# endernewton/tf-faster-rcnn

Measured on NVIDIA H100. Metric: images/sec, higher is better.
Workload: dtype f16x3 (fp32-grade: fp16 hi/lo split of both operands, 3 wgmma f16 MMAs per product, fp32 accumulate)

## Files before the change

include/frcnn_b200.h:

```cpp
#ifndef FRCNN_B200_H_
#define FRCNN_B200_H_

#include <stddef.h>
#include <stdint.h>

#ifdef __cplusplus
extern "C" {
#endif

typedef enum {
  FRCNN_OK = 0,
  FRCNN_ERR_CUDA = -1,
  FRCNN_ERR_ARG = -2,
  FRCNN_ERR_NO_DEVICE = -3,
  FRCNN_ERR_DRIVER_ENTRY = -4,
  FRCNN_ERR_CAPACITY = -5
} frcnn_status;

#define FRCNN_NMS_PLUS_ONE 1u
#define FRCNN_NMS_INCLUSIVE 2u
#define FRCNN_NMS_SKIP_DEGENERATE 4u
#define FRCNN_NMS_MODE_CPU_NMS (FRCNN_NMS_PLUS_ONE | FRCNN_NMS_INCLUSIVE)
#define FRCNN_NMS_MODE_GPU_NMS (FRCNN_NMS_PLUS_ONE)
#define FRCNN_NMS_MODE_TF (FRCNN_NMS_SKIP_DEGENERATE)
// ... 21 lines not shown

typedef struct frcnn_conv_plan frcnn_conv_plan;
#define FRCNN_CONV_F16X3 0
#define FRCNN_CONV_TF32X3 1
#define FRCNN_CONV_F16X1 2

typedef struct {
  const float* in_dev;
  const void* w_hi_dev;
  const void* w_lo_dev;
  const float* scale_dev;
  const float* shift_dev;
  const float* residual_dev;
  float* out_dev;
  int n, h, w, cin;
  int cout, kh, kw, stride;
  int pad_t, pad_l;
  int ho, wo;
  int act;
  int block_n;
  int kb_per_chunk;
  int split_k;
  int impl;
  float out_mult;
  const float* in2_dev;
  int cin2;
  float* mean_dev;
  int mean_hw;
} frcnn_conv_desc;

int frcnn_conv_plan_create(frcnn_conv_plan** out, const frcnn_conv_desc* d);
int frcnn_conv_plan_run(const frcnn_conv_plan* p, void* stream);
int frcnn_conv_plan_geometry(const frcnn_conv_desc* d, int sm_count, int* out16);
int frcnn_conv_plan_info(const frcnn_conv_plan* p, int* block_n, int* tile_n, int* tile_h, int* tile_w,
                         int* grid_m, int* grid_n, int* splits, int* smem_bytes);
int frcnn_conv_plan_set_trace(frcnn_conv_plan* p, long long* trace_dev);
void frcnn_conv_plan_destroy(frcnn_conv_plan* p);
int frcnn_debug_watchdog(unsigned int* out16, int reset);

int frcnn_pack_conv_weights(const float* w_hwio_dev, void* w_hi_dev, void* w_lo_dev, int kh, int kw,
                            int cin, int cout, int wexp, void* stream);
int frcnn_pack_conv_weights_tf32(const float* w_hwio_dev, float* w_hi_dev, float* w_lo_dev, int kh, int kw,
                                 int cin, int cout, void* stream);

int frcnn_conv_first(const float* in_dev, const float* w_hwio_dev, const float* scale_dev,
                     const float* shift_dev, float* out_dev, int n, int h, int w, int cout, int k,
                     int stride, int pad_t, int pad_l, int ho, int wo, int act, void* stream);
int frcnn_depthwise3x3(const float* in_dev, const float* w_dev, const float* scale_dev,
                       const float* shift_dev, float* out_dev, int n, int h, int w, int c, int stride,
                       int pad_t, int pad_l, int ho, int wo, int act, void* stream);
int frcnn_max_pool(const float* in_dev, float* out_dev, int n, int h, int w, int c, int k, int stride,
                   int pad_t, int pad_l, int ho, int wo, int pad_is_neg_inf, void* stream);
int frcnn_spatial_mean(const float* in_dev, float* out_dev, int r, int hw, int c, void* stream);

int frcnn_preprocess(const unsigned char* img_dev, int h0, int w0, const double* means3, double fx, double fy,
                     float* blob_dev, int H, int W, void* stream);
int frcnn_preprocess_hflip(const unsigned char* img_dev, int h0, int w0, const double* means3, double fx, double fy,
                           float* blob_dev, int H, int W, void* stream);


int frcnn_rpn_decode(const float* rpn_out_dev, int ld, int delta_col, const float* base_anchors_dev, int num_anchors,
                     int batch, int fh, int fw, int feat_stride, float im_h, float im_w, float* scores_dev,
                     float* props_dev, void* stream);
size_t frcnn_sort_workspace_bytes(int n);
int frcnn_sort_desc(const float* keys_dev, int n, int batch, int* order_dev, float* sorted_keys_dev, void* workspace_dev,
                    size_t workspace_bytes, void* stream);
// ... 73 lines not shown
```

tf_faster_rcnn_b200/_native.py:

```python
import ctypes as C
import os

_HERE = os.path.dirname(os.path.abspath(__file__))
LIB_PATH = os.path.join(_HERE, "libfrcnn_b200_wd.so" if os.environ.get("FRCNN_LIB_VARIANT") == "wd" else "libfrcnn_b200.so")

NMS_PLUS_ONE, NMS_INCLUSIVE, NMS_SKIP_DEGENERATE = 1, 2, 4
NMS_MODE_CPU_NMS = NMS_PLUS_ONE | NMS_INCLUSIVE
NMS_MODE_GPU_NMS = NMS_PLUS_ONE
NMS_MODE_TF = NMS_SKIP_DEGENERATE
ACT_NONE, ACT_RELU, ACT_RELU6 = 0, 1, 2
CONV_F16X3, CONV_TF32X3, CONV_F16X1 = 0, 1, 2
SOFT_NMS_METHODS = {"linear": 0, "gaussian": 1, "hard": 2}
AUG_MAX_VIEWS = 16
BOX_VOTE_METHODS = {"ID": 0, "AVG": 1, "IOU_AVG": 2, "GENERALIZED_AVG": 3, "QUASI_SUM": 4, "TEMP_AVG": 5}
ROI_ALIGN_MAX_SAMPLING = 16
ROI_MAX_POOLED = 16

vp, ci, cf, cu, sz = C.c_void_p, C.c_int, C.c_float, C.c_uint, C.c_size_t
ip, fp = C.POINTER(C.c_int), C.POINTER(C.c_float)


class ConvDesc(C.Structure):
    _fields_ = [("in_dev", vp), ("w_hi_dev", vp), ("w_lo_dev", vp), ("scale_dev", vp), ("shift_dev", vp),
                ("residual_dev", vp), ("out_dev", vp),
                ("n", ci), ("h", ci), ("w", ci), ("cin", ci), ("cout", ci), ("kh", ci), ("kw", ci), ("stride", ci),
                ("pad_t", ci), ("pad_l", ci), ("ho", ci), ("wo", ci), ("act", ci), ("block_n", ci), ("kb_per_chunk", ci), ("split_k", ci),
                ("impl", ci), ("out_mult", cf), ("in2_dev", vp), ("cin2", ci), ("mean_dev", vp), ("mean_hw", ci)]


SIGNATURES = {
    "frcnn_version": (ci, []),
    "frcnn_last_error": (ci, [C.c_char_p, sz]),
    "frcnn_check_device": (ci, [ci]),
    "frcnn_zero_async": (ci, [vp, sz, vp]),
    "frcnn_graph_begin": (ci, [vp]),
    "frcnn_graph_end": (ci, [vp, C.POINTER(vp)]),
    "frcnn_graph_launch": (ci, [vp, vp]),
    "frcnn_graph_destroy": (None, [vp]),
    "frcnn_nms_host": (ci, [ip, ip, fp, ci, ci, cf, ci, cu]),
    "frcnn_nms_sorted_dev": (ci, [vp, ci, cf, cu, ci, vp, vp, vp]),
    "frcnn_conv_plan_create": (ci, [C.POINTER(vp), C.POINTER(ConvDesc)]),
    "frcnn_conv_plan_run": (ci, [vp, vp]),
    "frcnn_conv_plan_geometry": (ci, [C.POINTER(ConvDesc), ci, ip]),
    "frcnn_conv_plan_info": (ci, [vp, ip, ip, ip, ip, ip, ip, ip, ip]),
    "frcnn_conv_plan_set_trace": (ci, [vp, vp]),
    "frcnn_conv_plan_destroy": (None, [vp]),
    "frcnn_debug_watchdog": (ci, [C.POINTER(C.c_uint), ci]),
    "frcnn_pack_conv_weights": (ci, [vp, vp, vp, ci, ci, ci, ci, ci, vp]),
    "frcnn_pack_conv_weights_tf32": (ci, [vp, vp, vp, ci, ci, ci, ci, vp]),
    "frcnn_conv_first": (ci, [vp, vp, vp, vp, vp, ci, ci, ci, ci, ci, ci, ci, ci, ci, ci, ci, vp]),
    "frcnn_depthwise3x3": (ci, [vp, vp, vp, vp, vp, ci, ci, ci, ci, ci, ci, ci, ci, ci, ci, vp]),
    "frcnn_max_pool": (ci, [vp, vp, ci, ci, ci, ci, ci, ci, ci, ci, ci, ci, ci, vp]),
    "frcnn_spatial_mean": (ci, [vp, vp, ci, ci, ci, vp]),
    "frcnn_preprocess": (ci, [vp, ci, ci, C.POINTER(C.c_double), C.c_double, C.c_double, vp, ci, ci, vp]),
    "frcnn_rpn_decode": (ci, [vp, ci, ci, vp, ci, ci, ci, ci, ci, cf, cf, vp, vp, vp]),
    "frcnn_sort_workspace_bytes": (sz, [ci]),
    "frcnn_sort_desc": (ci, [vp, ci, ci, vp, vp, vp, sz, vp]),
    "frcnn_proposals": (ci, [vp, vp, vp, ci, ci, ci, ci, cf, cu, vp, vp, vp, vp, vp]),
    "frcnn_crop_pool": (ci, [vp, ci, ci, ci, ci, vp, ci, ci, ci, vp, vp]),
    "frcnn_roi_align": (ci, [vp, ci, ci, ci, ci, vp, ci, ci, cf, ci, ci, vp, vp]),
    "frcnn_roi_pool": (ci, [vp, ci, ci, ci, ci, vp, ci, ci, cf, vp, vp]),
    "frcnn_cls_finish": (ci, [vp, ci, ci, ci, fp, fp, vp, vp, vp, vp]),
    "frcnn_bbox_decode": (ci, [vp, vp, ci, ci, ci, vp, vp, vp]),
    "frcnn_detect_post_workspace_bytes": (sz, [ci, ci, ci]),
    "frcnn_detect_regions_workspace_bytes": (ci, [ci, ci, ci, C.POINTER(sz)]),
    "frcnn_detect_post": (ci, [vp, vp, vp, ci, ci, ci, cf, cf, cu, ci, ci, vp, vp, ci, vp, vp, vp, vp, sz, vp]),
    "frcnn_soft_nms_host": (ci, [fp, ip, ip, fp, ci, ci, ci, cf, cf, cf, ci]),
    "frcnn_detect_post_soft": (ci, [vp, vp, vp, ci, ci, ci, cf, ci, cf, cf, cf, ci, ci, vp, vp, ci, vp, vp, vp, vp, sz, vp]),
    "frcnn_detect_features": (ci, [vp, vp, vp, ci, ci, ci, ci, ci, vp, vp, vp]),
    "frcnn_detect_regions": (ci, [vp, vp, vp, vp, vp, ci, ci, ci, ci, cf, cu, cf, ci, ci, vp, vp, vp, vp, sz, vp, vp, vp, vp, vp, vp, vp,
                                  vp, vp]),
    "frcnn_regions_attr_embed": (ci, [vp, ci, ci, ci, vp, vp, ci, vp, ci, vp, vp]),
    "frcnn_attr_finish": (ci, [vp, ci, ci, ci, ci, vp, vp, vp, vp, vp]),
    "frcnn_boxes_to_rois": (ci, [vp, vp, vp, ci, ci, vp, vp, vp]),
    "frcnn_preprocess_hflip": (ci, [vp, ci, ci, C.POINTER(C.c_double), C.c_double, C.c_double, vp, ci, ci, vp]),
    "frcnn_aug_union": (ci, [C.POINTER(vp), C.POINTER(vp), C.POINTER(vp), ip, ip, ci, ci, ci, vp, vp, vp, vp, vp]),
# ... 34 lines not shown
```

tf_faster_rcnn_b200/csrc/conv_gemm.cu:

```cuda
#include <cuda_fp16.h>
#include "common.cuh"
#include "../../include/frcnn_b200.h"
#include <stdlib.h>
#include <string.h>

namespace frcnn {

constexpr int BLOCK_M = 128;
constexpr int BLOCK_K = 32;
constexpr int A_TILE_BYTES = BLOCK_M * BLOCK_K * 4;
constexpr int NUM_CONSUMERS = 256;
constexpr int NUM_THREADS = NUM_CONSUMERS + 128;
constexpr int REGS_PRODUCER = 40, REGS_CONSUMER = 232;
constexpr int STAGES = 3;

struct ConvKernelParams {
  float* out;
  const float* residual;
  const float* scale;
  const float* shift;
  int cout, ho, wo, nimg;
  int tn, th, tw;
  int tiles_h, tiles_w;
  int kh, kw, cin, stride, pad_t, pad_l;
  int act;
  int a_box_bytes;
  int kb_per_split;
  int m_tiles, n_tiles, total_units, n_full, splits;
  int raster_n;
  float* ws;
  long long* trace;
  int num_kb_total;
  int cin2;
  float* mean_out;
  float* mean_ws;
  int mean_hw, mean_segs, mean_ld;
};

#ifdef FRCNN_WATCHDOG
#define FRCNN_TRACE(slot, kbv)                                                              \
  do {                                                                                      \
    if (p.trace && blockIdx.x == 0 && (kbv) < 64) p.trace[(kbv) * 8 + (slot)] = clock64(); \
  } while (0)
#else
#define FRCNN_TRACE(slot, kbv) do { } while (0)
#endif

template <int MODE> struct KTraits {
  static constexpr bool TF32 = MODE == FRCNN_CONV_TF32X3;
  static constexpr bool X1 = MODE == FRCNN_CONV_F16X1;
  static constexpr int BOXES = TF32 ? 1 : 2;
  static constexpr int A_BYTES = BOXES * A_TILE_BYTES;
  static constexpr float LO_SCALE = TF32 ? 1.f : 0.00048828125f;
};
template <int BN> constexpr int b_plane_bytes() { return BN * 128; }
template <int BN, int MODE> constexpr int stage_bytes() { return KTraits<MODE>::A_BYTES + 2 * b_plane_bytes<BN>(); }
template <int BN, int MODE> constexpr int smem_bytes() {
  return STAGES * stage_bytes<BN, MODE>() + 1024  + 64 ;
}
constexpr int MEAN_COLS = 64, MEAN_LD = MEAN_COLS + 2;
constexpr int MEAN_SMEM = BLOCK_M * MEAN_LD * 4;
static_assert(smem_bytes<128, FRCNN_CONV_F16X3>() + MEAN_SMEM <= 227 * 1024, "ring exceeds the sm_90 shared-memory limit per block");

struct Unit {
  int w0, h0, n0, nblk, z, kb0, num_kb, slot;
};
__device__ __forceinline__ Unit decode_unit(const ConvKernelParams& p, int u, int num_kb_total) {
  Unit t;
  int tile;
  if (u < p.n_full) { tile = u; t.z = 0; t.slot = -1; }
  else { const int v = u - p.n_full; t.slot = v / p.splits; t.z = v - t.slot * p.splits; tile = p.n_full + t.slot; }
  int mt;
  if (p.raster_n) { t.nblk = tile % p.n_tiles; mt = tile / p.n_tiles; }
  else { mt = tile % p.m_tiles; t.nblk = tile / p.m_tiles; }
  const int tile_w = mt % p.tiles_w;
  const int tile_h = (mt / p.tiles_w) % p.tiles_h;
  const int tile_n = mt / (p.tiles_w * p.tiles_h);
  t.w0 = tile_w * p.tw; t.h0 = tile_h * p.th; t.n0 = tile_n * p.tn;
  if (t.slot < 0) { t.kb0 = 0; t.num_kb = num_kb_total; }
  else { t.kb0 = t.z * p.kb_per_split; t.num_kb = min(p.kb_per_split, num_kb_total - t.kb0); }
  return t;
}

template <int ACT>
__device__ __forceinline__ float apply_act(float a) {
  if (ACT == FRCNN_ACT_RELU) return fmaxf(a, 0.f);
  if (ACT == FRCNN_ACT_RELU6) return fminf(fmaxf(a, 0.f), 6.f);
  return a;
}

template <bool RES, int ACT>
__device__ __forceinline__ float2 finish2(const float2 v, const float2 sc, const float2 sh, const float2 r) {
  float2 y;
  y.x = __fadd_rn(__fmul_rn(v.x, sc.x), sh.x); y.y = __fadd_rn(__fmul_rn(v.y, sc.y), sh.y);
  if (RES) { y.x = __fadd_rn(y.x, r.x); y.y = __fadd_rn(y.y, r.y); }
  y.x = apply_act<ACT>(y.x); y.y = apply_act<ACT>(y.y);
  return y;
}

constexpr int EPI_CHUNK = 8;
template <int BN, bool RES, int ACT>
__device__ __forceinline__ void epilogue_vec(const ConvKernelParams& p, const float (&acc)[BN / 2], const int cbase,
                                             const int pix0, const int pix1) {
  const int cout = p.cout;
  constexpr int NJ = BN / 8;
  constexpr int CH = NJ < EPI_CHUNK ? NJ : EPI_CHUNK;
  static_assert(NJ % CH == 0, "chunking");
  const float* const res0 = RES ? p.residual + (size_t)(pix0 >= 0 ? pix0 : 0) * cout : nullptr;
  const float* const res1 = RES ? p.residual + (size_t)(pix1 >= 0 ? pix1 : 0) * cout : nullptr;
#pragma unroll
  for (int j0 = 0; j0 < NJ; j0 += CH) {
    if (cbase + 8 * j0 >= cout) break;
    float2 sc[CH], sh[CH], r0[CH], r1[CH];
#pragma unroll
// ... 158 lines not shown
  constexpr int kStage = stage_bytes<BN, MODE>();
  constexpr int kPlane = b_plane_bytes<BN>();
  constexpr int NACC = BN / 2;
  static_assert(BN == 64 || BN == 128, "block_n");

  extern __shared__ uint8_t smem_raw[];
  uint8_t* smem = reinterpret_cast<uint8_t*>((reinterpret_cast<uintptr_t>(smem_raw) + 1023) & ~uintptr_t(1023));
  uint64_t* full = reinterpret_cast<uint64_t*>(smem + STAGES * kStage);
  uint64_t* empty = full + STAGES;

  const int warp = threadIdx.x >> 5;
  const int lane = threadIdx.x & 31;
  const int num_kb_total = p.num_kb_total;

  if (threadIdx.x == NUM_CONSUMERS) {
    tma_prefetch_desc(&tmA); tma_prefetch_desc(&tmBhi); tma_prefetch_desc(&tmBlo);
    if (p.cin2) tma_prefetch_desc(&tmA2);
    for (int s = 0; s < STAGES; ++s) { mbar_init(&full[s], 1); mbar_init(&empty[s], NUM_CONSUMERS); }
    mbar_fence_init();
  }
  __syncthreads();
  pdl_launch_dependents();
  pdl_wait();

  if (warp >= NUM_CONSUMERS / 32) {
    reg_dec<REGS_PRODUCER>();
    if (warp == NUM_CONSUMERS / 32 && lane == 0) {
      const int cchunks = p.cin / BLOCK_K;
      const int total1 = p.kh * p.kw * cchunks;
      const int cchunks2 = p.cin2 / BLOCK_K;
      const uint32_t tx = (uint32_t)(T::BOXES * p.a_box_bytes + (T::X1 ? 1 : 2) * kPlane);
      int s = 0; uint32_t ph = 0, kbt = 0;
      for (int u = blockIdx.x; u < p.total_units; u += gridDim.x) {
        const Unit t = decode_unit(p, u, num_kb_total);
#pragma unroll 1
        for (int kb = 0; kb < t.num_kb; ++kb, ++kbt) {
          MBAR_WAIT(&empty[s], ph ^ 1u, 4, kbt);
          uint8_t* st = smem + s * kStage;
          mbar_expect_tx(&full[s], tx);
#pragma unroll
          for (int i = 0; i < T::BOXES; ++i) {
            const int g32 = (t.kb0 + kb) * T::BOXES + i;
            int tap = g32 / cchunks, kc = g32 - tap * cchunks;
            const CUtensorMap* ma = &tmA;
            if (g32 >= total1) {
              tap = 0;
              if (cchunks2) { ma = &tmA2; kc = min(g32 - total1, cchunks2); }
              else kc = cchunks;
            }
            const int r = tap / p.kw, sx = tap - r * p.kw;
            tma_load_4d(st + i * A_TILE_BYTES, ma, &full[s], kc * BLOCK_K, t.w0 * p.stride + sx - p.pad_l,
                        t.h0 * p.stride + r - p.pad_t, t.n0);
          }
          const int kcoord = (t.kb0 + kb) * T::BOXES * BLOCK_K;
          tma_load_2d(st + T::A_BYTES, &tmBhi, &full[s], kcoord, t.nblk * BN);
          if (!T::X1) tma_load_2d(st + T::A_BYTES + kPlane, &tmBlo, &full[s], kcoord, t.nblk * BN);
          FRCNN_TRACE(0, kbt);
          if (++s == STAGES) { s = 0; ph ^= 1u; }
        }
      }
    }
    return;
  }

  reg_inc<REGS_CONSUMER>();
  const int wg = warp >> 2;
  const int q4 = lane & 3;
  const int r0 = wg * 64 + (warp & 3) * 16 + (lane >> 2);
  const uint32_t swz = (uint32_t)(lane >> 2);
  uint32_t aoff[4][2];
#pragma unroll
  for (int j = 0; j < 4; ++j)
#pragma unroll
    for (int h = 0; h < 2; ++h) {
      const int ch = T::TF32 ? j * 8 + h * 4 + q4 : (j & 1) * 16 + h * 8 + 2 * q4;
      const int box = T::TF32 ? 0 : j >> 1;
      aoff[j][h] = (uint32_t)(box * A_TILE_BYTES + r0 * 128) + ((((uint32_t)ch >> 2) ^ swz) << 4) + (((uint32_t)ch & 3u) << 2);
    }
  const uint32_t smem0 = smem_u32(smem);
  int s = 0; uint32_t ph = 0, kbt = 0;
  for (int u = blockIdx.x; u < p.total_units; u += gridDim.x) {
    const Unit t = decode_unit(p, u, num_kb_total);
    float acc[NACC], part[NACC];
#pragma unroll
    for (int i = 0; i < NACC; ++i) { acc[i] = 0.f; part[i] = 0.f; }
#pragma unroll 1
    for (int kb = 0; kb < t.num_kb; ++kb, ++kbt) {
      MBAR_WAIT(&full[s], ph, 1, kbt);
      if (threadIdx.x == 0) FRCNN_TRACE(1, kbt);
      const uint32_t sa = smem0 + (uint32_t)(s * kStage);
      uint32_t ahi[4][4], alo[4][4];
#pragma unroll
      for (int j = 0; j < 4; ++j) {
#pragma unroll
        for (int f = 0; f < 4; ++f) {
          const uint32_t addr = sa + aoff[j][f >> 1] + ((f & 1) ? 1024u : 0u);
          if (T::TF32) {
            float x;
            asm volatile("ld.shared.f32 %0, [%1];" : "=f"(x) : "r"(addr));
            const float hi = to_tf32(x);
            ahi[j][f] = __float_as_uint(hi);
            alo[j][f] = __float_as_uint(to_tf32_fast(__fsub_rn(x, hi)));
          } else {
            float2 x;
            asm volatile("ld.shared.v2.f32 {%0, %1}, [%2];" : "=f"(x.x), "=f"(x.y) : "r"(addr));
            const uint32_t h = pack_f16x2_rn(x.x, x.y);
            const float2 fh = __half22float2(*reinterpret_cast<const __half2*>(&h));
            ahi[j][f] = h;
            alo[j][f] = T::X1 ? 0u : pack_f16x2_rn(__fmul_rn(__fsub_rn(x.x, fh.x), 2048.f), __fmul_rn(__fsub_rn(x.y, fh.y), 2048.f));
          }
        }
      }
      const uint64_t bhi = wgmma_sw128_desc(sa + (uint32_t)T::A_BYTES);
      const uint64_t blo = wgmma_sw128_desc(sa + (uint32_t)(T::A_BYTES + kPlane));
#pragma unroll
      for (int i = 0; i < NACC; ++i) reg_fence(part[i]);
      wgmma_fence();
#pragma unroll
      for (int j = 0; j < 4; ++j) wgmma_rs<BN, MODE>(part, ahi[j], bhi + 2u * j, j > 0 ? 1u : 0u);
      wgmma_commit();
      wgmma_wait_all();
#pragma unroll
      for (int i = 0; i < NACC; ++i) { reg_fence(part[i]); acc[i] = __fadd_rn(acc[i], part[i]); }
      if (!T::X1) {
        wgmma_fence();
#pragma unroll
        for (int j = 0; j < 4; ++j) {
          wgmma_rs<BN, MODE>(part, alo[j], bhi + 2u * j, j > 0 ? 1u : 0u);
          wgmma_rs<BN, MODE>(part, ahi[j], blo + 2u * j, 1u);
        }
        wgmma_commit();
        wgmma_wait_all();
#pragma unroll
        for (int i = 0; i < NACC; ++i) { reg_fence(part[i]); acc[i] = __fmaf_rn(part[i], T::LO_SCALE, acc[i]); }
      }
      mbar_arrive(&empty[s]);
      if (threadIdx.x == 0) FRCNN_TRACE(2, kbt);
      if (++s == STAGES) { s = 0; ph ^= 1u; }
    }
    epilogue_tile<BN>(p, t, acc, r0, q4, reinterpret_cast<float*>(full + 8));
  }
}

template <int BN>
__global__ void __launch_bounds__(256)
tail_reduce_kernel(const ConvKernelParams p) {
  pdl_launch_dependents();
  pdl_wait();
  constexpr int RPB = 256 / (BN / 4);
  constexpr int GROUPS = BLOCK_M / RPB;
  const int slot = blockIdx.x / GROUPS, rgroup = blockIdx.x % GROUPS;
  const int tile = p.n_full + slot;
  const int mt = p.raster_n ? tile / p.n_tiles : tile % p.m_tiles, nblk = p.raster_n ? tile % p.n_tiles : tile / p.m_tiles;
  const int tile_w = mt % p.tiles_w, tile_h = (mt / p.tiles_w) % p.tiles_h, tile_n = mt / (p.tiles_w * p.tiles_h);
  const int rows_img = p.th * p.tw;
  constexpr int C4 = BN / 4;
  static_assert(256 % C4 == 0, "each thread keeps one fixed channel group");
  const float* base = p.ws + (size_t)slot * p.splits * (size_t)(BLOCK_M * BN);
  const bool vec_ok = (p.cout & 3) == 0;
  const int cg = threadIdx.x % C4;
  const int c = nblk * BN + cg * 4;
  if (c >= p.cout) return;
  const float4 sc4 = __ldg(reinterpret_cast<const float4*>(p.scale + c)), sh4 = __ldg(reinterpret_cast<const float4*>(p.shift + c));
  const float sc[4] = {sc4.x, sc4.y, sc4.z, sc4.w}, sh[4] = {sh4.x, sh4.y, sh4.z, sh4.w};
  {
    const int row = rgroup * RPB + threadIdx.x / C4;
    const int dn = row / rows_img, rem = row % rows_img;
    const int n = tile_n * p.tn + dn, h = tile_h * p.th + rem / p.tw, w = tile_w * p.tw + rem % p.tw;
    if (row >= p.tn * rows_img || n >= p.nimg || h >= p.ho || w >= p.wo) return;
    const size_t o = ((((size_t)n * p.ho + h) * p.wo + w)) * p.cout + c;
    float4 rv = make_float4(0.f, 0.f, 0.f, 0.f);
// ... 217 lines not shown
  FRCNN_REQUIRE(bn == 64 || bn == 128, "block_n must be 64 or 128");
  g->bn = bn;
  g->n_tiles = cdiv(d->cout, bn);
  g->tiles = g->m_tiles * g->n_tiles;
  FRCNN_REQUIRE(g->tiles <= 0x3fffffffL, "too many tiles");
  long n_tail = 0; int splits = 1;
  const int num_kb = g->num_kb;
  const int max_split = num_kb * ks / 8 < 8 ? num_kb * ks / 8 : 8;
  if (d->split_k > 1) {
    n_tail = g->tiles; splits = d->split_k;
  } else if (d->split_k == 0 && max_split >= 2) {
    const long rem = g->tiles % sms;
    if (g->tiles <= sms / 2) { if (num_kb * ks >= 16) { n_tail = g->tiles; splits = (int)(sms / g->tiles); } }
    else if (g->tiles > sms && rem > 0 && rem <= sms / 2 && num_kb * ks >= 48) { n_tail = rem; splits = (int)(sms / rem); }
    if (splits > max_split) splits = max_split;
    if (splits < 2) { n_tail = 0; splits = 1; }
  }
  int kbs = cdiv(num_kb, splits);
  splits = cdiv(num_kb, kbs);
  if (splits < 2 || (d->cout & 3) != 0 || mean) { n_tail = 0; splits = 1; kbs = num_kb; }
  FRCNN_REQUIRE(splits <= 64, "bad split_k");
  g->n_tail = n_tail; g->splits = splits; g->kbs = kbs;
  g->total_units = (g->tiles - n_tail) + n_tail * splits;
  FRCNN_REQUIRE(g->total_units <= 0x7fffffffL, "too many work units");
  g->grid = (int)(g->total_units < sms ? g->total_units : sms);
  {
    const char* e = getenv("FRCNN_CONV_RASTER");
    const double a_bytes = (double)d->n * d->h * d->w * (d->cin + d->cin2) * 4.0, b_bytes = (double)d->cout * ktot * 4.0;
    g->raster_n = (e && (e[0] == 'm' || e[0] == 'n')) ? (e[0] == 'n') : (a_bytes > b_bytes && g->n_tiles > 1);
  }
  return OK;
}

extern "C" int frcnn_conv_plan_geometry(const frcnn_conv_desc* d, int sm_count, int* out16) {
  FRCNN_REQUIRE(d && out16, "null argument");
  Geometry g;
  int rc = decide_geometry(d, sm_count, &g);
  if (rc) return rc;
  const int v[16] = {g.bn, g.tn, g.th, g.tw, (int)g.m_tiles, g.n_tiles, (int)g.tiles, (int)g.n_tail, g.splits, g.kbs,
                     (int)g.total_units, g.grid, g.num_kb, g.kpc, g.tiles_h, g.tiles_w};
  for (int i = 0; i < 16; ++i) out16[i] = v[i];
  return OK;
}

extern "C" int frcnn_conv_plan_create(frcnn_conv_plan** out, const frcnn_conv_desc* d) {
  FRCNN_REQUIRE(out && d, "null argument");
  FRCNN_REQUIRE(d->in_dev && d->w_hi_dev && d->w_lo_dev && (d->mean_hw ? d->mean_dev != nullptr : d->out_dev != nullptr),
                "null device pointer");
  FRCNN_REQUIRE(d->cin2 == 0 || d->in2_dev, "cin2=%d without in2_dev", d->cin2);
  int sms = 132;
  { int dev = 0; cudaDeviceProp pr; if (cudaGetDevice(&dev) == cudaSuccess && cudaGetDeviceProperties(&pr, dev) == cudaSuccess && pr.multiProcessorCount > 0) sms = pr.multiProcessorCount; }
  Geometry g;
  int grc = decide_geometry(d, sms, &g);
  if (grc) return grc;
  frcnn_conv_plan* p = (frcnn_conv_plan*)aligned_alloc(64, (sizeof(frcnn_conv_plan) + 63) / 64 * 64);
  if (!p) { set_error("out of host memory"); return ERR_ARG; }
  memset(p, 0, sizeof(*p));
  const int bn = g.bn;
  {
    uint64_t dims[4] = {(uint64_t)d->cin, (uint64_t)g.w, (uint64_t)g.h, (uint64_t)g.n};
    uint64_t strides[3] = {(uint64_t)d->cin * 4, (uint64_t)g.w * d->cin * 4, (uint64_t)g.h * g.w * d->cin * 4};
    uint32_t box[4] = {(uint32_t)BLOCK_K, (uint32_t)(g.tw * d->stride), (uint32_t)(g.th * d->stride), (uint32_t)g.tn};
    uint32_t es[4] = {1, (uint32_t)d->stride, (uint32_t)d->stride, 1};
    int rc = encode_map(&p->tmA, d->in_dev, 4, dims, strides, box, es);
    if (rc) { free(p); return rc; }
    p->tmA2 = p->tmA;
    if (d->cin2 > 0) {
      uint64_t dims2[4] = {(uint64_t)d->cin2, (uint64_t)g.w, (uint64_t)g.h, (uint64_t)g.n};
      uint64_t strides2[3] = {(uint64_t)d->cin2 * 4, (uint64_t)g.w * d->cin2 * 4, (uint64_t)g.h * g.w * d->cin2 * 4};
      rc = encode_map(&p->tmA2, d->in2_dev, 4, dims2, strides2, box, es);
      if (rc) { free(p); return rc; }
    }
  }
  const bool f16 = d->impl != FRCNN_CONV_TF32X3;
  {
    const uint64_t ktot = (uint64_t)d->kh * d->kw * d->cin + d->cin2;
    uint64_t dims[2] = {ktot, (uint64_t)d->cout};
    uint64_t strides[1] = {ktot * (f16 ? 2 : 4)};
    uint32_t box[2] = {(uint32_t)(f16 ? 2 * BLOCK_K : BLOCK_K), (uint32_t)bn};
    uint32_t es[2] = {1, 1};
    const CUtensorMapDataType dt = f16 ? CU_TENSOR_MAP_DATA_TYPE_FLOAT16 : CU_TENSOR_MAP_DATA_TYPE_FLOAT32;
    const CUtensorMapSwizzle sw = CU_TENSOR_MAP_SWIZZLE_128B;
    int rc = encode_map(&p->tmBhi, d->w_hi_dev, 2, dims, strides, box, es, dt, sw);
    if (!rc) rc = encode_map(&p->tmBlo, d->w_lo_dev, 2, dims, strides, box, es, dt, sw);
    if (rc) { free(p); return rc; }
  }
  ConvKernelParams& k = p->kp;
  k.out = d->out_dev; k.residual = d->residual_dev;
  k.cout = d->cout; k.ho = g.ho; k.wo = g.wo; k.nimg = g.n;
  k.tn = g.tn; k.th = g.th; k.tw = g.tw; k.tiles_h = g.tiles_h; k.tiles_w = g.tiles_w;
  k.kh = d->kh; k.kw = d->kw; k.cin = d->cin; k.stride = d->stride; k.pad_t = d->pad_t; k.pad_l = d->pad_l;
  k.act = d->act;
  k.a_box_bytes = g.tn * g.th * g.tw * BLOCK_K * 4;
  k.trace = nullptr;
  k.num_kb_total = g.num_kb;
  k.m_tiles = (int)g.m_tiles; k.n_tiles = g.n_tiles;
  k.kb_per_split = g.kbs; k.splits = g.splits; k.n_full = (int)(g.tiles - g.n_tail);
  k.total_units = (int)g.total_units;
  k.raster_n = g.raster_n;
  k.cin2 = d->cin2;
  k.mean_out = d->mean_hw ? d->mean_dev : nullptr; k.mean_ws = nullptr; k.mean_hw = d->mean_hw; k.mean_ld = g.n_tiles * bn;
  k.mean_segs = d->mean_hw ? (g.tw < cdiv(g.tw - 1, d->mean_hw) + 1 ? g.tw : cdiv(g.tw - 1, d->mean_hw) + 1) : 0;
  k.ws = nullptr; p->ws = nullptr; p->eff = nullptr; p->mean_ws = nullptr; p->n_tail = (int)g.n_tail;
  {
    const int padded = g.n_tiles * bn;
    const float om = f16 ? (d->out_mult != 0.f ? d->out_mult : 1.f) : 1.f;
    cudaError_t e = cudaMalloc(&p->eff, (size_t)2 * padded * sizeof(float));
    if (e != cudaSuccess) { free(p); return cuda_fail(e, "epilogue vectors", __FILE__, __LINE__); }
    prep_epilogue_vectors_kernel<<<cdiv(padded, 256), 256>>>(d->scale_dev, d->shift_dev, om, d->cout, padded, p->eff, p->eff + padded);
    e = cudaGetLastError();
    if (e == cudaSuccess) e = cudaDeviceSynchronize();
    if (e != cudaSuccess) { cudaFree(p->eff); free(p); return cuda_fail(e, "prep_epilogue_vectors", __FILE__, __LINE__); }
    k.scale = p->eff; k.shift = p->eff + padded;
  }
  if (g.n_tail > 0) {
    cudaError_t e = cudaMalloc(&p->ws, (size_t)g.n_tail * g.splits * BLOCK_M * bn * sizeof(float));
    if (e != cudaSuccess) { cudaFree(p->eff); free(p); return cuda_fail(e, "split-tile workspace", __FILE__, __LINE__); }
    k.ws = p->ws;
  }
  if (d->mean_hw) {
    cudaError_t e = cudaMalloc(&p->mean_ws, (size_t)g.m_tiles * k.mean_segs * k.mean_ld * sizeof(float));
    if (e != cudaSuccess) { cudaFree(p->eff); free(p); return cuda_fail(e, "mean workspace", __FILE__, __LINE__); }
    k.mean_ws = p->mean_ws;
  }
  p->grid = dim3((unsigned)g.grid, 1, 1);
  p->block_n = bn;
  p->impl = f16 ? (d->impl == FRCNN_CONV_F16X1 ? FRCNN_CONV_F16X1 : FRCNN_CONV_F16X3) : FRCNN_CONV_TF32X3;
  p->stages = STAGES;
  p->smem = f16 ? (bn == 128 ? smem_bytes<128, FRCNN_CONV_F16X3>() : smem_bytes<64, FRCNN_CONV_F16X3>())
              : (bn == 128 ? smem_bytes<128, FRCNN_CONV_TF32X3>() : smem_bytes<64, FRCNN_CONV_TF32X3>());
  if (d->mean_hw) p->smem += MEAN_SMEM;
  *out = p;
  return OK;
}

// ... 49 lines not shown
```

Baseline: 261.8.

## Skip conv K-blocks whose filter taps fall entirely in padding

Per output tile, computes which kernel rows and columns touch any in-bounds input pixel and narrows the K-block range (plus per-block liveness checks) so the TMA producer and MMA consumer skip blocks that would load only zero padding. Enabled per plan only when the host-side count finds dead blocks. Removes wasted loads and wgmma work on border tiles, at the cost of extra index arithmetic per K-block and per unit in both producer and consumer loops.

After: 264.5, median of 6. 1.0% higher.

```diff
diff --git a/include/frcnn_b200.h b/include/frcnn_b200.h
--- a/include/frcnn_b200.h
+++ b/include/frcnn_b200.h
@@ -77,6 +77,7 @@
 int frcnn_conv_plan_create(frcnn_conv_plan** out, const frcnn_conv_desc* d);
 int frcnn_conv_plan_run(const frcnn_conv_plan* p, void* stream);
 int frcnn_conv_plan_geometry(const frcnn_conv_desc* d, int sm_count, int* out16);
+int frcnn_conv_plan_live_kblocks(const frcnn_conv_desc* d, int sm_count, long* live, long* total);
 int frcnn_conv_plan_info(const frcnn_conv_plan* p, int* block_n, int* tile_n, int* tile_h, int* tile_w,
                          int* grid_m, int* grid_n, int* splits, int* smem_bytes);
 int frcnn_conv_plan_set_trace(frcnn_conv_plan* p, long long* trace_dev);
diff --git a/tf_faster_rcnn_b200/_native.py b/tf_faster_rcnn_b200/_native.py
--- a/tf_faster_rcnn_b200/_native.py
+++ b/tf_faster_rcnn_b200/_native.py
@@ -42,6 +42,7 @@
     "frcnn_conv_plan_create": (ci, [C.POINTER(vp), C.POINTER(ConvDesc)]),
     "frcnn_conv_plan_run": (ci, [vp, vp]),
     "frcnn_conv_plan_geometry": (ci, [C.POINTER(ConvDesc), ci, ip]),
+    "frcnn_conv_plan_live_kblocks": (ci, [C.POINTER(ConvDesc), ci, C.POINTER(C.c_long), C.POINTER(C.c_long)]),
     "frcnn_conv_plan_info": (ci, [vp, ip, ip, ip, ip, ip, ip, ip, ip]),
     "frcnn_conv_plan_set_trace": (ci, [vp, vp]),
     "frcnn_conv_plan_destroy": (None, [vp]),
diff --git a/tf_faster_rcnn_b200/csrc/conv_gemm.cu b/tf_faster_rcnn_b200/csrc/conv_gemm.cu
--- a/tf_faster_rcnn_b200/csrc/conv_gemm.cu
+++ b/tf_faster_rcnn_b200/csrc/conv_gemm.cu
@@ -23,6 +23,7 @@
   int tn, th, tw;
   int tiles_h, tiles_w;
   int kh, kw, cin, stride, pad_t, pad_l;
+  int h, w;
   int act;
   int a_box_bytes;
   int kb_per_split;
@@ -32,6 +33,7 @@
   long long* trace;
   int num_kb_total;
   int cin2;
+  int pad_skip;
   float* mean_out;
   float* mean_ws;
   int mean_hw, mean_segs, mean_ld;
@@ -64,8 +66,44 @@
 
 struct Unit {
   int w0, h0, n0, nblk, z, kb0, num_kb, slot;
+  uint32_t live;
+  int kb_begin, kb_end;
 };
-__device__ __forceinline__ Unit decode_unit(const ConvKernelParams& p, int u, int num_kb_total) {
+
+__host__ __device__ __forceinline__ uint32_t live_taps(int o0, int n, int k, int stride, int pad, int extent) {
+  if (k > 16) return 0xffffu;
+  uint32_t m = 0;
+  for (int i = 0; i < k; ++i) {
+    const int y0 = o0 * stride + i - pad;
+    const int j = y0 >= 0 ? 0 : (stride - 1 - y0) / stride;
+    if (j < n && y0 + j * stride < extent) m |= 1u << i;
+  }
+  return m;
+}
+
+__host__ __device__ __forceinline__ bool kblock_live(const ConvKernelParams& p, const Unit& t, int kb, int boxes) {
+  if (t.live == ~0u) return true;
+  const int cchunks = p.cin / BLOCK_K, total1 = p.kh * p.kw * cchunks;
+  for (int i = 0; i < boxes; ++i) {
+    const int g32 = kb * boxes + i;
+    if (g32 >= total1) {
+      if (p.cin2) return true;
+      continue;
+    }
+    const int tap = g32 / cchunks, r = tap / p.kw, s = tap - r * p.kw;
+    if (r >= 16 || s >= 16 || ((t.live >> r) & (t.live >> (16 + s)) & 1u)) return true;
+  }
+  return false;
+}
+
+__host__ __device__ __forceinline__ int live_kblock_count(const ConvKernelParams& p, const Unit& t, int boxes) {
+  if (t.live == ~0u) return t.kb_end > t.kb_begin ? t.kb_end - t.kb_begin : 0;
+  int n = 0;
+  for (int kb = t.kb_begin; kb < t.kb_end; ++kb) n += kblock_live(p, t, kb, boxes);
+  return n;
+}
+
+__host__ __device__ __forceinline__ Unit decode_unit(const ConvKernelParams& p, int u, int num_kb_total, int boxes) {
   Unit t;
   int tile;
   if (u < p.n_full) { tile = u; t.z = 0; t.slot = -1; }
@@ -78,7 +116,30 @@
   const int tile_n = mt / (p.tiles_w * p.tiles_h);
   t.w0 = tile_w * p.tw; t.h0 = tile_h * p.th; t.n0 = tile_n * p.tn;
   if (t.slot < 0) { t.kb0 = 0; t.num_kb = num_kb_total; }
-  else { t.kb0 = t.z * p.kb_per_split; t.num_kb = min(p.kb_per_split, num_kb_total - t.kb0); }
+  else { t.kb0 = t.z * p.kb_per_split; t.num_kb = p.kb_per_split < num_kb_total - t.kb0 ? p.kb_per_split : num_kb_total - t.kb0; }
+  if (!p.pad_skip) {
+    t.live = ~0u; t.kb_begin = t.kb0; t.kb_end = t.kb0 + t.num_kb;
+    return t;
+  }
+  const uint32_t live_r = live_taps(t.h0, p.th, p.kh, p.stride, p.pad_t, p.h);
+  const uint32_t live_s = live_taps(t.w0, p.tw, p.kw, p.stride, p.pad_l, p.w);
+  int r_lo = -1, r_hi = -1;
+  bool gap = false;
+  for (int r = 0; r < p.kh; ++r)
+    if (r >= 16 || ((live_r >> r) & 1u)) {
+      if (r_lo < 0) r_lo = r;
+      else if (r_hi != r - 1) gap = true;
+      r_hi = r;
+    }
+  const uint32_t all_s = p.kw >= 16 ? 0xffffu : (1u << p.kw) - 1u;
+  const int per_row = p.kw * (p.cin / BLOCK_K), total1 = p.kh * per_row;
+  int box_lo = 0, box_hi = 0;
+  if (r_lo >= 0 && live_s != 0) { box_lo = r_lo * per_row; box_hi = (r_hi + 1) * per_row; }
+  if (p.cin2) { if (box_hi == 0) box_lo = total1; box_hi = total1 + p.cin2 / BLOCK_K; }
+  const int kb_lo = box_lo / boxes, kb_hi = (box_hi + boxes - 1) / boxes;
+  t.kb_begin = t.kb0 > kb_lo ? t.kb0 : kb_lo;
+  t.kb_end = t.kb0 + t.num_kb < kb_hi ? t.kb0 + t.num_kb : kb_hi;
+  t.live = !gap && (live_s & all_s) == all_s ? ~0u : live_r | live_s << 16;
   return t;
 }
 
@@ -304,15 +365,16 @@
       const uint32_t tx = (uint32_t)(T::BOXES * p.a_box_bytes + (T::X1 ? 1 : 2) * kPlane);
       int s = 0; uint32_t ph = 0, kbt = 0;
       for (int u = blockIdx.x; u < p.total_units; u += gridDim.x) {
-        const Unit t = decode_unit(p, u, num_kb_total);
+        const Unit t = decode_unit(p, u, num_kb_total, T::BOXES);
 #pragma unroll 1
-        for (int kb = 0; kb < t.num_kb; ++kb, ++kbt) {
+        for (int kb = t.kb_begin; kb < t.kb_end; ++kb) {
+          if (!kblock_live(p, t, kb, T::BOXES)) continue;
           MBAR_WAIT(&empty[s], ph ^ 1u, 4, kbt);
           uint8_t* st = smem + s * kStage;
           mbar_expect_tx(&full[s], tx);
 #pragma unroll
           for (int i = 0; i < T::BOXES; ++i) {
-            const int g32 = (t.kb0 + kb) * T::BOXES + i;
+            const int g32 = kb * T::BOXES + i;
             int tap = g32 / cchunks, kc = g32 - tap * cchunks;
             const CUtensorMap* ma = &tmA;
             if (g32 >= total1) {
@@ -324,11 +386,12 @@
             tma_load_4d(st + i * A_TILE_BYTES, ma, &full[s], kc * BLOCK_K, t.w0 * p.stride + sx - p.pad_l,
                         t.h0 * p.stride + r - p.pad_t, t.n0);
           }
-          const int kcoord = (t.kb0 + kb) * T::BOXES * BLOCK_K;
+          const int kcoord = kb * T::BOXES * BLOCK_K;
           tma_load_2d(st + T::A_BYTES, &tmBhi, &full[s], kcoord, t.nblk * BN);
           if (!T::X1) tma_load_2d(st + T::A_BYTES + kPlane, &tmBlo, &full[s], kcoord, t.nblk * BN);
           FRCNN_TRACE(0, kbt);
           if (++s == STAGES) { s = 0; ph ^= 1u; }
+          ++kbt;
         }
       }
     }
@@ -352,12 +415,13 @@
   const uint32_t smem0 = smem_u32(smem);
   int s = 0; uint32_t ph = 0, kbt = 0;
   for (int u = blockIdx.x; u < p.total_units; u += gridDim.x) {
-    const Unit t = decode_unit(p, u, num_kb_total);
+    const Unit t = decode_unit(p, u, num_kb_total, T::BOXES);
     float acc[NACC], part[NACC];
 #pragma unroll
     for (int i = 0; i < NACC; ++i) { acc[i] = 0.f; part[i] = 0.f; }
+    const int num_live = live_kblock_count(p, t, T::BOXES);
 #pragma unroll 1
-    for (int kb = 0; kb < t.num_kb; ++kb, ++kbt) {
+    for (int kb = 0; kb < num_live; ++kb) {
       MBAR_WAIT(&full[s], ph, 1, kbt);
       if (threadIdx.x == 0) FRCNN_TRACE(1, kbt);
       const uint32_t sa = smem0 + (uint32_t)(s * kStage);
@@ -409,6 +473,7 @@
       mbar_arrive(&empty[s]);
       if (threadIdx.x == 0) FRCNN_TRACE(2, kbt);
       if (++s == STAGES) { s = 0; ph ^= 1u; }
+      ++kbt;
     }
     epilogue_tile<BN>(p, t, acc, r0, q4, reinterpret_cast<float*>(full + 8));
   }
@@ -703,6 +768,44 @@
   return OK;
 }
 
+static void unit_params(const frcnn_conv_desc* d, const Geometry& g, ConvKernelParams* k) {
+  k->cout = d->cout; k->ho = g.ho; k->wo = g.wo; k->nimg = g.n;
+  k->tn = g.tn; k->th = g.th; k->tw = g.tw; k->tiles_h = g.tiles_h; k->tiles_w = g.tiles_w;
+  k->kh = d->kh; k->kw = d->kw; k->cin = d->cin; k->stride = d->stride; k->pad_t = d->pad_t; k->pad_l = d->pad_l;
+  k->h = g.h; k->w = g.w;
+  k->num_kb_total = g.num_kb;
+  k->m_tiles = (int)g.m_tiles; k->n_tiles = g.n_tiles;
+  k->kb_per_split = g.kbs; k->splits = g.splits; k->n_full = (int)(g.tiles - g.n_tail);
+  k->total_units = (int)g.total_units;
+  k->raster_n = g.raster_n;
+  k->cin2 = d->cin2;
+}
+
+static void count_kblocks(ConvKernelParams* k, int impl, long* live, long* total) {
+  const int boxes = impl != FRCNN_CONV_TF32X3 ? 2 : 1;
+  k->pad_skip = 1;
+  long nl = 0, nt = 0;
+  for (int u = 0; u < k->total_units; ++u) {
+    const Unit t = decode_unit(*k, u, k->num_kb_total, boxes);
+    nl += live_kblock_count(*k, t, boxes);
+    nt += t.num_kb;
+  }
+  k->pad_skip = nl < nt;
+  *live = nl; *total = nt;
+}
+
+extern "C" int frcnn_conv_plan_live_kblocks(const frcnn_conv_desc* d, int sm_count, long* live, long* total) {
+  FRCNN_REQUIRE(d && live && total, "null argument");
+  Geometry g;
+  int rc = decide_geometry(d, sm_count, &g);
+  if (rc) return rc;
+  ConvKernelParams k;
+  memset(&k, 0, sizeof(k));
+  unit_params(d, g, &k);
+  count_kblocks(&k, d->impl, live, total);
+  return OK;
+}
+
 extern "C" int frcnn_conv_plan_create(frcnn_conv_plan** out, const frcnn_conv_desc* d) {
   FRCNN_REQUIRE(out && d, "null argument");
   FRCNN_REQUIRE(d->in_dev && d->w_hi_dev && d->w_lo_dev && (d->mean_hw ? d->mean_dev != nullptr : d->out_dev != nullptr),
@@ -746,19 +849,15 @@
     if (rc) { free(p); return rc; }
   }
   ConvKernelParams& k = p->kp;
+  unit_params(d, g, &k);
+  {
+    long live, total;
+    count_kblocks(&k, d->impl, &live, &total);
+  }
   k.out = d->out_dev; k.residual = d->residual_dev;
-  k.cout = d->cout; k.ho = g.ho; k.wo = g.wo; k.nimg = g.n;
-  k.tn = g.tn; k.th = g.th; k.tw = g.tw; k.tiles_h = g.tiles_h; k.tiles_w = g.tiles_w;
-  k.kh = d->kh; k.kw = d->kw; k.cin = d->cin; k.stride = d->stride; k.pad_t = d->pad_t; k.pad_l = d->pad_l;
   k.act = d->act;
   k.a_box_bytes = g.tn * g.th * g.tw * BLOCK_K * 4;
   k.trace = nullptr;
-  k.num_kb_total = g.num_kb;
-  k.m_tiles = (int)g.m_tiles; k.n_tiles = g.n_tiles;
-  k.kb_per_split = g.kbs; k.splits = g.splits; k.n_full = (int)(g.tiles - g.n_tail);
-  k.total_units = (int)g.total_units;
-  k.raster_n = g.raster_n;
-  k.cin2 = d->cin2;
   k.mean_out = d->mean_hw ? d->mean_dev : nullptr; k.mean_ws = nullptr; k.mean_hw = d->mean_hw; k.mean_ld = g.n_tiles * bn;
   k.mean_segs = d->mean_hw ? (g.tw < cdiv(g.tw - 1, d->mean_hw) + 1 ? g.tw : cdiv(g.tw - 1, d->mean_hw) + 1) : 0;
   k.ws = nullptr; p->ws = nullptr; p->eff = nullptr; p->mean_ws = nullptr; p->n_tail = (int)g.n_tail;
```

## Skip conv K-blocks whose filter taps read only zero padding

Applied to the files above, without the earlier changes.

Computes per output tile which kernel taps touch any in-bounds input pixel, and has both the TMA producer and the MMA consumer skip K-blocks made up entirely of padding-only taps. Plan creation counts live and total K-blocks on the host and turns skipping on only when some can be skipped; a query entry point exposes these counts. This removes loads and MMAs that only multiply zero padding on border tiles, at the cost of extra per-unit bookkeeping in both warps and a risk of producer/consumer count mismatch.

Result: faster. 263.0 before, 266.7 after (median of 6 runs) (+1.4%).

```diff
diff --git a/include/frcnn_b200.h b/include/frcnn_b200.h
--- a/include/frcnn_b200.h
+++ b/include/frcnn_b200.h
@@ -77,6 +77,7 @@
 int frcnn_conv_plan_create(frcnn_conv_plan** out, const frcnn_conv_desc* d);
 int frcnn_conv_plan_run(const frcnn_conv_plan* p, void* stream);
 int frcnn_conv_plan_geometry(const frcnn_conv_desc* d, int sm_count, int* out16);
+int frcnn_conv_plan_live_kblocks(const frcnn_conv_desc* d, int sm_count, long long* live, long long* total);
 int frcnn_conv_plan_info(const frcnn_conv_plan* p, int* block_n, int* tile_n, int* tile_h, int* tile_w,
                          int* grid_m, int* grid_n, int* splits, int* smem_bytes);
 int frcnn_conv_plan_set_trace(frcnn_conv_plan* p, long long* trace_dev);
diff --git a/tf_faster_rcnn_b200/_native.py b/tf_faster_rcnn_b200/_native.py
--- a/tf_faster_rcnn_b200/_native.py
+++ b/tf_faster_rcnn_b200/_native.py
@@ -42,6 +42,7 @@
     "frcnn_conv_plan_create": (ci, [C.POINTER(vp), C.POINTER(ConvDesc)]),
     "frcnn_conv_plan_run": (ci, [vp, vp]),
     "frcnn_conv_plan_geometry": (ci, [C.POINTER(ConvDesc), ci, ip]),
+    "frcnn_conv_plan_live_kblocks": (ci, [C.POINTER(ConvDesc), ci, C.POINTER(C.c_longlong), C.POINTER(C.c_longlong)]),
     "frcnn_conv_plan_info": (ci, [vp, ip, ip, ip, ip, ip, ip, ip, ip]),
     "frcnn_conv_plan_set_trace": (ci, [vp, vp]),
     "frcnn_conv_plan_destroy": (None, [vp]),
diff --git a/tf_faster_rcnn_b200/csrc/conv_gemm.cu b/tf_faster_rcnn_b200/csrc/conv_gemm.cu
--- a/tf_faster_rcnn_b200/csrc/conv_gemm.cu
+++ b/tf_faster_rcnn_b200/csrc/conv_gemm.cu
@@ -35,6 +35,8 @@
   float* mean_out;
   float* mean_ws;
   int mean_hw, mean_segs, mean_ld;
+  int h, w;
+  int pad_skip;
 };
 
 #ifdef FRCNN_WATCHDOG
@@ -65,7 +67,7 @@
 struct Unit {
   int w0, h0, n0, nblk, z, kb0, num_kb, slot;
 };
-__device__ __forceinline__ Unit decode_unit(const ConvKernelParams& p, int u, int num_kb_total) {
+__host__ __device__ __forceinline__ Unit decode_unit(const ConvKernelParams& p, int u, int num_kb_total) {
   Unit t;
   int tile;
   if (u < p.n_full) { tile = u; t.z = 0; t.slot = -1; }
@@ -78,8 +80,70 @@
   const int tile_n = mt / (p.tiles_w * p.tiles_h);
   t.w0 = tile_w * p.tw; t.h0 = tile_h * p.th; t.n0 = tile_n * p.tn;
   if (t.slot < 0) { t.kb0 = 0; t.num_kb = num_kb_total; }
-  else { t.kb0 = t.z * p.kb_per_split; t.num_kb = min(p.kb_per_split, num_kb_total - t.kb0); }
+  else { t.kb0 = t.z * p.kb_per_split; t.num_kb = num_kb_total - t.kb0 < p.kb_per_split ? num_kb_total - t.kb0 : p.kb_per_split; }
   return t;
+}
+
+
+__host__ __device__ __forceinline__ bool line_reads_map(int first, int n, int step, int size) {
+  if (first >= size) return false;
+  if (first >= 0) return true;
+  const int j = (-first + step - 1) / step;
+  return j < n && first + j * step < size;
+}
+
+__host__ __device__ __forceinline__ unsigned long long unit_live_taps(const ConvKernelParams& p, const Unit& t) {
+  const int taps = p.kh * p.kw;
+  if (taps > 64) return ~0ull;
+  unsigned long long cols = 0, m = 0;
+#pragma unroll 1
+  for (int s = 0; s < p.kw; ++s)
+    if (line_reads_map(t.w0 * p.stride + s - p.pad_l, p.tw, p.stride, p.w)) cols |= 1ull << s;
+#pragma unroll 1
+  for (int r = 0; r < p.kh; ++r)
+    if (line_reads_map(t.h0 * p.stride + r - p.pad_t, p.th, p.stride, p.h)) m |= cols << (r * p.kw);
+  return m == (taps == 64 ? ~0ull : (1ull << taps) - 1) ? ~0ull : m;
+}
+
+struct KCursor {
+  int g, tap, kc;
+};
+__host__ __device__ __forceinline__ KCursor kcursor(const ConvKernelParams& p, int kb, int boxes) {
+  const int cchunks = p.cin / BLOCK_K;
+  KCursor c;
+  c.g = kb * boxes; c.tap = c.g / cchunks; c.kc = c.g - c.tap * cchunks;
+  return c;
+}
+
+__host__ __device__ __forceinline__ bool kblock_live(const ConvKernelParams& p, unsigned long long live, KCursor& c, int boxes) {
+  const int cchunks = p.cin / BLOCK_K, total1 = p.kh * p.kw * cchunks;
+  bool any = false;
+  for (int i = 0; i < boxes; ++i) {
+    if (c.g < total1) any |= ((live >> c.tap) & 1ull) != 0;
+    else any |= p.cin2 != 0;
+    ++c.g;
+    if (++c.kc == cchunks) { c.kc = 0; ++c.tap; }
+  }
+  return any;
+}
+
+__host__ __device__ __forceinline__ int unit_live_kblocks(const ConvKernelParams& p, const Unit& t, unsigned long long live,
+                                                          int boxes) {
+  if (live == ~0ull) return t.num_kb;
+  const int cchunks = p.cin / BLOCK_K;
+  if (p.cin2 == 0 && cchunks % boxes == 0) {
+    const int kpt = cchunks / boxes, kb1 = t.kb0 + t.num_kb;
+    int n = 0;
+#pragma unroll 1
+    for (int tap = t.kb0 / kpt; tap * kpt < kb1; ++tap)
+      if ((live >> tap) & 1ull) n += (kb1 < (tap + 1) * kpt ? kb1 : (tap + 1) * kpt) - (t.kb0 > tap * kpt ? t.kb0 : tap * kpt);
+    return n;
+  }
+  KCursor c = kcursor(p, t.kb0, boxes);
+  int n = 0;
+#pragma unroll 1
+  for (int kb = 0; kb < t.num_kb; ++kb) n += kblock_live(p, live, c, boxes);
+  return n;
 }
 
 template <int ACT>
@@ -305,14 +369,17 @@
       int s = 0; uint32_t ph = 0, kbt = 0;
       for (int u = blockIdx.x; u < p.total_units; u += gridDim.x) {
         const Unit t = decode_unit(p, u, num_kb_total);
+        const unsigned long long live = p.pad_skip ? unit_live_taps(p, t) : ~0ull;
+        KCursor c = kcursor(p, t.kb0, T::BOXES);
 #pragma unroll 1
-        for (int kb = 0; kb < t.num_kb; ++kb, ++kbt) {
+        for (int kb = t.kb0; kb < t.kb0 + t.num_kb; ++kb) {
+          if (live != ~0ull && !kblock_live(p, live, c, T::BOXES)) continue;
           MBAR_WAIT(&empty[s], ph ^ 1u, 4, kbt);
           uint8_t* st = smem + s * kStage;
           mbar_expect_tx(&full[s], tx);
 #pragma unroll
           for (int i = 0; i < T::BOXES; ++i) {
-            const int g32 = (t.kb0 + kb) * T::BOXES + i;
+            const int g32 = kb * T::BOXES + i;
             int tap = g32 / cchunks, kc = g32 - tap * cchunks;
             const CUtensorMap* ma = &tmA;
             if (g32 >= total1) {
@@ -324,10 +391,11 @@
             tma_load_4d(st + i * A_TILE_BYTES, ma, &full[s], kc * BLOCK_K, t.w0 * p.stride + sx - p.pad_l,
                         t.h0 * p.stride + r - p.pad_t, t.n0);
           }
-          const int kcoord = (t.kb0 + kb) * T::BOXES * BLOCK_K;
+          const int kcoord = kb * T::BOXES * BLOCK_K;
           tma_load_2d(st + T::A_BYTES, &tmBhi, &full[s], kcoord, t.nblk * BN);
           if (!T::X1) tma_load_2d(st + T::A_BYTES + kPlane, &tmBlo, &full[s], kcoord, t.nblk * BN);
           FRCNN_TRACE(0, kbt);
+          ++kbt;
           if (++s == STAGES) { s = 0; ph ^= 1u; }
         }
       }
@@ -353,11 +421,12 @@
   int s = 0; uint32_t ph = 0, kbt = 0;
   for (int u = blockIdx.x; u < p.total_units; u += gridDim.x) {
     const Unit t = decode_unit(p, u, num_kb_total);
+    const int n_live = p.pad_skip ? unit_live_kblocks(p, t, unit_live_taps(p, t), T::BOXES) : t.num_kb;
     float acc[NACC], part[NACC];
 #pragma unroll
     for (int i = 0; i < NACC; ++i) { acc[i] = 0.f; part[i] = 0.f; }
 #pragma unroll 1
-    for (int kb = 0; kb < t.num_kb; ++kb, ++kbt) {
+    for (int kb = 0; kb < n_live; ++kb, ++kbt) {
       MBAR_WAIT(&full[s], ph, 1, kbt);
       if (threadIdx.x == 0) FRCNN_TRACE(1, kbt);
       const uint32_t sa = smem0 + (uint32_t)(s * kStage);
@@ -692,6 +761,45 @@
   return OK;
 }
 
+static void kernel_shape(const frcnn_conv_desc* d, const Geometry& g, ConvKernelParams* k) {
+  k->cout = d->cout; k->ho = g.ho; k->wo = g.wo; k->nimg = g.n; k->h = g.h; k->w = g.w;
+  k->tn = g.tn; k->th = g.th; k->tw = g.tw; k->tiles_h = g.tiles_h; k->tiles_w = g.tiles_w;
+  k->kh = d->kh; k->kw = d->kw; k->cin = d->cin; k->stride = d->stride; k->pad_t = d->pad_t; k->pad_l = d->pad_l;
+  k->act = d->act;
+  k->a_box_bytes = g.tn * g.th * g.tw * BLOCK_K * 4;
+  k->num_kb_total = g.num_kb;
+  k->m_tiles = (int)g.m_tiles; k->n_tiles = g.n_tiles;
+  k->kb_per_split = g.kbs; k->splits = g.splits; k->n_full = (int)(g.tiles - g.n_tail);
+  k->total_units = (int)g.total_units;
+  k->raster_n = g.raster_n;
+  k->cin2 = d->cin2;
+  k->mean_hw = d->mean_hw; k->mean_ld = g.n_tiles * g.bn;
+  k->mean_segs = d->mean_hw ? (g.tw < cdiv(g.tw - 1, d->mean_hw) + 1 ? g.tw : cdiv(g.tw - 1, d->mean_hw) + 1) : 0;
+}
+
+static void count_kblocks(const ConvKernelParams& k, int impl, long long* live, long long* total) {
+  const int boxes = impl == FRCNN_CONV_TF32X3 ? 1 : 2;
+  long long nl = 0, nt = 0;
+  for (int u = 0; u < k.total_units; ++u) {
+    const Unit t = decode_unit(k, u, k.num_kb_total);
+    nl += unit_live_kblocks(k, t, unit_live_taps(k, t), boxes);
+    nt += t.num_kb;
+  }
+  *live = nl; *total = nt;
+}
+
+extern "C" int frcnn_conv_plan_live_kblocks(const frcnn_conv_desc* d, int sm_count, long long* live, long long* total) {
+  FRCNN_REQUIRE(d && live && total, "null argument");
+  Geometry g;
+  int rc = decide_geometry(d, sm_count, &g);
+  if (rc) return rc;
+  ConvKernelParams k;
+  memset(&k, 0, sizeof(k));
+  kernel_shape(d, g, &k);
+  count_kblocks(k, d->impl, live, total);
+  return OK;
+}
+
 extern "C" int frcnn_conv_plan_geometry(const frcnn_conv_desc* d, int sm_count, int* out16) {
   FRCNN_REQUIRE(d && out16, "null argument");
   Geometry g;
@@ -746,21 +854,15 @@
     if (rc) { free(p); return rc; }
   }
   ConvKernelParams& k = p->kp;
+  kernel_shape(d, g, &k);
+  {
+    long long live = 0, total = 0;
+    count_kblocks(k, d->impl, &live, &total);
+    k.pad_skip = live < total;
+  }
   k.out = d->out_dev; k.residual = d->residual_dev;
-  k.cout = d->cout; k.ho = g.ho; k.wo = g.wo; k.nimg = g.n;
-  k.tn = g.tn; k.th = g.th; k.tw = g.tw; k.tiles_h = g.tiles_h; k.tiles_w = g.tiles_w;
-  k.kh = d->kh; k.kw = d->kw; k.cin = d->cin; k.stride = d->stride; k.pad_t = d->pad_t; k.pad_l = d->pad_l;
-  k.act = d->act;
-  k.a_box_bytes = g.tn * g.th * g.tw * BLOCK_K * 4;
   k.trace = nullptr;
-  k.num_kb_total = g.num_kb;
-  k.m_tiles = (int)g.m_tiles; k.n_tiles = g.n_tiles;
-  k.kb_per_split = g.kbs; k.splits = g.splits; k.n_full = (int)(g.tiles - g.n_tail);
-  k.total_units = (int)g.total_units;
-  k.raster_n = g.raster_n;
-  k.cin2 = d->cin2;
-  k.mean_out = d->mean_hw ? d->mean_dev : nullptr; k.mean_ws = nullptr; k.mean_hw = d->mean_hw; k.mean_ld = g.n_tiles * bn;
-  k.mean_segs = d->mean_hw ? (g.tw < cdiv(g.tw - 1, d->mean_hw) + 1 ? g.tw : cdiv(g.tw - 1, d->mean_hw) + 1) : 0;
+  k.mean_out = d->mean_hw ? d->mean_dev : nullptr; k.mean_ws = nullptr;
   k.ws = nullptr; p->ws = nullptr; p->eff = nullptr; p->mean_ws = nullptr; p->n_tail = (int)g.n_tail;
   {
     const int padded = g.n_tiles * bn;
```
